# nv-tlabs/DefTet

Measured on AMD Instinct MI355X. Metric: M tet-point tests/s (fwd+bwd) at res=70, 100k queries, higher is better.
Workload: dtype f32

## Files before the change

deftet_amd/csrc/point_in_tet.hip:

```cpp
#pragma clang fp contract(off)

#include <stdlib.h>

#include <algorithm>
#include <type_traits>
#include <vector>

#include "common.hpp"

namespace deftet {
namespace pit {

constexpr float kBig = 1048576.0f;
constexpr float kTau = 1.0f / 128.0f;
constexpr float kMargin = 1.0f / 64.0f;
constexpr float kWMin = 9.3132257e-10f;
constexpr int kMiss = 0x7F7F7F7F;
constexpr int kMaxG = 112;
constexpr int kMaxBins = 15 * 1024;
constexpr int kHitOverflow = -2;

constexpr int kHitPad = 64;
__host__ __device__ inline int hit_pad(int B) { return (B + kHitPad - 1) / kHitPad * kHitPad; }
__host__ __device__ inline size_t hit_cnt_off(int B, int T) { return (size_t)B * T * 2; }
// ... 215 lines not shown
    const float cells = fmaxf(4096.0f, (float)Q * (1.0f / 32.0f)) * layers / fmaxf((float)Q, 1.0f);
    return cells >= 2.0e9f ? 0x7FFFFFFF : (int)cells;
}
__device__ __forceinline__ bool wide_tet(int cx0, int cx1, int cy0, int cy1, int cz0, int cz1, const Grid &g)
{
    return (cx1 - cx0 + 1) * ((cy1 - cy0 + 1) * (cz1 - cz0 + 1)) > g.wide;
}

__device__ __forceinline__ bool query_regular(float x, float y, float z)
{
    return fabsf(x) <= kBig && fabsf(y) <= kBig && fabsf(z) <= kBig;
}

__host__ __device__ inline int table_pitch(int G) { return G + 3; }
__device__ __forceinline__ unsigned table_off(int cz, int cx, int cy, int Gx, int Gp)
{
    return (unsigned)((cz * (Gx + 1) + cx) * Gp + cy);
}

__global__ __launch_bounds__(256) void k_query_bbox(const float *__restrict__ pts, int Q, float *part, int *counters,
                                                    int *result, int nB, long long nQ)
{
    __shared__ float sh[4][6];
    const int b = blockIdx.y;
    {
        const long long nblk = (long long)gridDim.x * gridDim.y, bid = (long long)blockIdx.y * gridDim.x + blockIdx.x;
        const long long i = bid * blockDim.x + threadIdx.x, stride = nblk * blockDim.x;
        if (i < nB * 8) counters[i] = 0;
        for (long long j = i; j < nQ; j += stride) result[j] = kMiss;
    }
    const float *p = pts + (size_t)b * Q * 3;
    float lo[3] = {INFINITY, INFINITY, INFINITY}, hi[3] = {-INFINITY, -INFINITY, -INFINITY};
    constexpr int kBoxKeep = 8;
    const int stride = gridDim.x * blockDim.x;
    for (int q0 = blockIdx.x * blockDim.x + threadIdx.x; q0 < Q; q0 += stride * kBoxKeep) {
        float x[kBoxKeep], y[kBoxKeep], z[kBoxKeep];
#pragma unroll
        for (int k = 0; k < kBoxKeep; ++k) {
            const float *pq = p + (size_t)min(q0 + k * stride, Q - 1) * 3;
            x[k] = pq[0]; y[k] = pq[1]; z[k] = pq[2];
        }
#pragma unroll
        for (int k = 0; k < kBoxKeep; ++k)
            if (query_regular(x[k], y[k], z[k])) {
                lo[0] = fminf(lo[0], x[k]); lo[1] = fminf(lo[1], y[k]); lo[2] = fminf(lo[2], z[k]);
                hi[0] = fmaxf(hi[0], x[k]); hi[1] = fmaxf(hi[1], y[k]); hi[2] = fmaxf(hi[2], z[k]);
            }
    }
#pragma unroll
    for (int off = 32; off > 0; off >>= 1) {
#pragma unroll
        for (int k = 0; k < 3; ++k) {
            lo[k] = fminf(lo[k], __shfl_xor(lo[k], off));
            hi[k] = fmaxf(hi[k], __shfl_xor(hi[k], off));
        }
    }
    const int w = threadIdx.x >> 6;
    if ((threadIdx.x & 63) == 0) {
#pragma unroll
        for (int k = 0; k < 3; ++k) { sh[w][k] = lo[k]; sh[w][3 + k] = hi[k]; }
    }
    __syncthreads();
    if (threadIdx.x < 6) {
        const int k = threadIdx.x;
        float v = sh[0][k];
        for (int i = 1; i < 4; ++i) v = k < 3 ? fminf(v, sh[i][k]) : fmaxf(v, sh[i][k]);
        part[((size_t)b * kBoxBlocks + blockIdx.x) * 6 + k] = v;
    }
}

__device__ __forceinline__ int2 shape_block(int pin)
{
    if (!pin) return make_int2(blockIdx.y, blockIdx.x);
    const int L = blockIdx.y * gridDim.x + blockIdx.x, nB = gridDim.y;
    return make_int2(L % nB, L / nB);
}
static inline int pin_shapes(int Q) { return (size_t)Q * 36 <= ((size_t)4 << 20); }

constexpr int kMaxRowBlocks = 256;
#ifndef PIT_ROWTILE
#define PIT_ROWTILE 2048
#endif
constexpr int kRowTile = PIT_ROWTILE;
constexpr int kLocalKeep = kRowTile / 256;
constexpr int kSub = 8;
constexpr int kParts = 4;
constexpr int kSubPerPart = kSub / kParts;
constexpr int kMaxBin1 = kMaxG * kSub;

template <bool HINT>
__global__ __launch_bounds__(256) void k_slab_local(const float *__restrict__ pts, int Q, const float *__restrict__ bboxPart,
                                                    float *gparam, int G, int Gx, int nblk, int nblkPad, int chunkQ,
                                                    float4 *localQ, int *pre, int *counters, int *irregQ,
                                                    const float *__restrict__ boxIn, float *partOut, int *irrCnt, int *result)
{
    __shared__ int hist[kMaxBin1 + 1];
    __shared__ int wtot[4];
    __shared__ int s_irr, s_out;
    __shared__ float s_box[4][6];
    const int b = blockIdx.y, blk = blockIdx.x, R1 = G * kSub, tid = threadIdx.x;
    const int q0 = blk * chunkQ, q1 = min(Q, q0 + chunkQ);
    const bool keep = chunkQ <= kRowTile;
    float3 kp[kLocalKeep];
    if (keep) {
#pragma unroll
        for (int k = 0; k < kLocalKeep; ++k) {
            const float *p = pts + ((size_t)b * Q + max(min(q0 + tid + k * 256, q1 - 1), 0)) * 3;
            kp[k] = make_float3(p[0], p[1], p[2]);
        }
    }
    if (HINT) {
        for (int q = q0 + tid; q < q1; q += 256) result[(size_t)b * Q + q] = kMiss;
        if (tid == 0) { s_irr = 0; s_out = 0; }
    }
    const Grid g = HINT ? hint_grid(boxIn + (size_t)b * 6, G, Gx) : reduce_grid(bboxPart + (size_t)b * kBoxBlocks * 6, kBoxBlocks, G, Gx);
    float blo[3] = {INFINITY, INFINITY, INFINITY}, bhi[3] = {-INFINITY, -INFINITY, -INFINITY};
    auto box_add = [&](float x, float y, float z) {
        if (HINT && query_regular(x, y, z)) {
            blo[0] = fminf(blo[0], x); blo[1] = fminf(blo[1], y); blo[2] = fminf(blo[2], z);
            bhi[0] = fmaxf(bhi[0], x); bhi[1] = fmaxf(bhi[1], y); bhi[2] = fmaxf(bhi[2], z);
        }
    };
    auto binned = [&](float x, float y, float z) { return HINT ? query_binned(x, y, z, g) : query_regular(x, y, z); };
    auto list_irregular = [&](int q, float x, float y, float z) {
        if (HINT) {
            irregQ[(size_t)b * Q + q0 + atomicAdd(&s_irr, 1)] = q;
            if (query_regular(x, y, z)) atomicAdd(&s_out, 1);
        } else {
            irregQ[(size_t)b * Q + atomicAdd(&counters[b * 4 + 1], 1)] = q;
        }
    };
    if (blk == 0 && tid == 0) {
        float *gp = gparam + b * kGridWords;
#pragma unroll
        for (int k = 0; k < 3; ++k) { gp[k] = g.o[k]; gp[3 + k] = g.inv[k]; gp[6 + k] = g.lo[k]; gp[9 + k] = g.hi[k]; gp[12 + k] = g.pe[k]; gp[15 + k] = g.cs[k]; }
        gp[18] = __int_as_float(wide_cells(g, Q, G, Gx));
        gp[19] = HINT ? 1.0f : 0.f;
    }
    for (int i = tid; i <= R1; i += 256) hist[i] = 0;
    __syncthreads();
    const float rcpG = 1.0f / (float)G;
    int kbin[kLocalKeep], krank[kLocalKeep];
    auto bin_of = [&](float x, float y, float z) {
        const int cy = cell_of(y, g.o[1], g.inv[1], G);
        return cell_of(z, g.o[2], g.inv[2], G) * kSub + (int)(((float)(cy * kSub) + 0.5f) * rcpG);
    };
    if (keep) {
#pragma unroll
        for (int k = 0; k < kLocalKeep; ++k) {
            const int q = q0 + tid + k * 256;
            kbin[k] = -1;
            if (q < q1) {
                box_add(kp[k].x, kp[k].y, kp[k].z);
                if (binned(kp[k].x, kp[k].y, kp[k].z)) {
                    kbin[k] = bin_of(kp[k].x, kp[k].y, kp[k].z);
                    krank[k] = atomicAdd(&hist[kbin[k]], 1);
                } else {
                    list_irregular(q, kp[k].x, kp[k].y, kp[k].z);
                }
            }
        }
    } else {
        for (int q = q0 + tid; q < q1; q += 256) {
            const float *p = pts + ((size_t)b * Q + q) * 3;
            const float x = p[0], y = p[1], z = p[2];
            box_add(x, y, z);
            if (binned(x, y, z)) atomicAdd(&hist[bin_of(x, y, z)], 1);
            else list_irregular(q, x, y, z);
        }
    }
    if (HINT) {
#pragma unroll
        for (int off = 32; off > 0; off >>= 1) {
#pragma unroll
            for (int k = 0; k < 3; ++k) {
                blo[k] = fminf(blo[k], __shfl_xor(blo[k], off));
                bhi[k] = fmaxf(bhi[k], __shfl_xor(bhi[k], off));
            }
        }
        if ((tid & 63) == 0) {
#pragma unroll
            for (int k = 0; k < 3; ++k) { s_box[tid >> 6][k] = blo[k]; s_box[tid >> 6][3 + k] = bhi[k]; }
        }
    }
    __syncthreads();
    if (HINT) {
        if (tid < 6) {
            float v = s_box[0][tid];
            for (int i = 1; i < 4; ++i) v = tid < 3 ? fminf(v, s_box[i][tid]) : fmaxf(v, s_box[i][tid]);
            partOut[((size_t)b * kMaxRowBlocks + blk) * 6 + tid] = v;
        }
        if (tid == 0) {
            irrCnt[b * kMaxRowBlocks + blk] = s_irr;
            irrCnt[(gridDim.y + b) * kMaxRowBlocks + blk] = s_out;
        }
    }
    {
        constexpr int kPer = (kMaxBin1 + 255) / 256;
        const int per = (R1 + 255) / 256, i0 = tid * per;
        int n[kPer], sum = 0;
#pragma unroll
        for (int j = 0; j < kPer; ++j) {
            n[j] = (j < per && i0 + j < R1) ? hist[i0 + j] : 0;
            sum += n[j];
        }
        int incl = sum;
        const int lane = tid & 63, w = tid >> 6;
#pragma unroll
        for (int off = 1; off < 64; off <<= 1) {
            const int t = __shfl_up(incl, off);
            if (lane >= off) incl += t;
        }
        if (lane == 63) wtot[w] = incl;
        __syncthreads();
        int run = incl - sum;
#pragma unroll
        for (int k = 0; k < 4; ++k)
            if (k < w) run += wtot[k];
        int *col = pre + (size_t)b * (R1 + 1) * nblkPad + blk;
#pragma unroll
        for (int j = 0; j < kPer; ++j)
            if (j < per && i0 + j < R1) {
                hist[i0 + j] = run;
                col[(size_t)(i0 + j) * nblkPad] = run;
                run += n[j];
            }
        if (tid == 255) col[(size_t)R1 * nblkPad] = run;
    }
    __syncthreads();
    float4 *dst = localQ + (size_t)b * Q + q0;
    if (keep) {
#pragma unroll
        for (int k = 0; k < kLocalKeep; ++k)
            if (kbin[k] >= 0) dst[hist[kbin[k]] + krank[k]] = make_float4(kp[k].x, kp[k].y, kp[k].z, __int_as_float(q0 + tid + k * 256));
    } else {
        for (int q = q0 + tid; q < q1; q += 256) {
            const float *p = pts + ((size_t)b * Q + q) * 3;
            const float x = p[0], y = p[1], z = p[2];
            if (binned(x, y, z)) dst[atomicAdd(&hist[bin_of(x, y, z)], 1)] = make_float4(x, y, z, __int_as_float(q));
        }
    }
}

#ifndef PIT_SORT_THREADS
#define PIT_SORT_THREADS 256
#endif
constexpr int kSortThreads = PIT_SORT_THREADS;
constexpr int kSortKeep = 1024 / kSortThreads;
constexpr int kRunsPer = kMaxRowBlocks / kSortThreads;
static_assert(kRunsPer * kSortThreads == kMaxRowBlocks && kSortThreads % 64 == 0, "every chunk run has a thread");
__global__ __launch_bounds__(kSortThreads) void k_slab_sort(const float4 *__restrict__ localQ, int Q, const float *__restrict__ gparam,
                                                            int G, int Gx, const int *__restrict__ pre, int nblk, int nblkPad,
                                                            int chunkQ, long long cellStride, int *table, float4 *sortedQ, int pin,
                                                            const float *__restrict__ boxPart, int nPart, int partStride, float *boxOut,
                                                            int hint, const int *__restrict__ irrCnt, int *irregQ, int *counters,
                                                            int *missOut)
{
    if (shape_block(pin).y == 0 && (boxOut || hint)) {
        const int b0 = shape_block(pin).x, nB = gridDim.y;
        if (boxOut && threadIdx.x < 64) {
            float lo[3], hi[3];
            reduce_box(boxPart + (size_t)b0 * partStride * 6, nPart, lo, hi);
            if (threadIdx.x == 0) {
#pragma unroll
                for (int k = 0; k < 3; ++k) { boxOut[b0 * 6 + k] = lo[k]; boxOut[b0 * 6 + 3 + k] = hi[k]; }
            }
        }
        if (hint && threadIdx.x < 64) {
            int n = 0, nOut = 0;
            for (int c = 0; c < nblk; ++c) {
                const int cnt = irrCnt[b0 * kMaxRowBlocks + c];
                nOut += irrCnt[(nB + b0) * kMaxRowBlocks + c];
                const int *src = irregQ + (size_t)b0 * Q + (size_t)c * chunkQ;
                for (int i = (int)threadIdx.x; i < cnt; i += 64) {
                    const int v = src[i];
                    irregQ[(size_t)b0 * Q + n + i] = v;
                }
                n += cnt;
            }
            if (threadIdx.x == 0) {
                counters[b0 * 4 + 0] = 0; counters[b0 * 4 + 1] = n; counters[b0 * 4 + 2] = 0; counters[b0 * 4 + 3] = 0;
#pragma unroll
                for (int k = 0; k < 4; ++k) counters[nB * 4 + b0 * 4 + k] = 0;
                if (missOut) missOut[b0] = nOut;
            }
        }
    }
    extern __shared__ __attribute__((aligned(16))) int cnt[];
    __shared__ int wsum[kSortThreads / 64], wsum2[kSortThreads / 64];
    __shared__ int runStart[kMaxRowBlocks + 1], runSrc[kMaxRowBlocks];
    const int2 sb = shape_block(pin);
    const int b = sb.x, cz = sb.y / kParts, part = sb.y % kParts, tid = threadIdx.x, lane = tid & 63, w = tid >> 6;
    const int GxP = Gx | 1;
    const int cyLo = (part * kSubPerPart * G + kSub - 1) / kSub, cyHi = ((part + 1) * kSubPerPart * G + kSub - 1) / kSub;
    const int nb = (cyHi - cyLo) * GxP, R1 = G * kSub;
    const int binLo = cz * kSub + part * kSubPerPart;
    PHASE_DECL;
    SPAN_MARK(0);
    int a[kRunsPer], len[kRunsPer], asum = 0, lsum = 0;
#pragma unroll
    for (int j = 0; j < kRunsPer; ++j) {
        const int r = tid * kRunsPer + j;
        a[j] = 0; len[j] = 0;
        if (r < nblk) {
            const int *row = pre + (size_t)b * (R1 + 1) * nblkPad;
            a[j] = row[(size_t)binLo * nblkPad + r];
            len[j] = row[(size_t)(binLo + kSubPerPart) * nblkPad + r] - a[j];
        }
        asum += a[j];
        lsum += len[j];
    }
    int s0, n;
    {
        int ia = asum, il = lsum;
#pragma unroll
        for (int off = 1; off < 64; off <<= 1) {
            const int ta = __shfl_up(ia, off), tl = __shfl_up(il, off);
            if (lane >= off) { ia += ta; il += tl; }
        }
        if (lane == 63) { wsum[w] = ia; wsum2[w] = il; }
        __syncthreads();
        int ta = 0, tl = 0, before = 0;
#pragma unroll
        for (int k = 0; k < kSortThreads / 64; ++k) {
            ta += wsum[k];
            tl += wsum2[k];
            if (k < w) before += wsum2[k];
        }
        s0 = ta;
        n = tl;
        int at = before + il - lsum;
#pragma unroll
        for (int j = 0; j < kRunsPer; ++j) {
            const int r = tid * kRunsPer + j;
            if (r < nblk) {
                runStart[r] = at;
                runSrc[r] = r * chunkQ + a[j];
            }
            at += len[j];
        }
        if (tid == 0) runStart[nblk] = n;
    }
    for (int i = tid; i < ((nb + 3) & ~3); i += kSortThreads) cnt[i] = 0;
    __syncthreads();
    const float ox = gparam[b * kGridWords + 0], oy = gparam[b * kGridWords + 1];
    const float ix = gparam[b * kGridWords + 3], iy = gparam[b * kGridWords + 4];
    const int s1 = s0 + n;
    const bool keep = n <= kSortThreads * kSortKeep;
    const float4 *src = localQ + (size_t)b * Q;
    auto source_of = [&](int i) {
        int lo = 0, hi = nblk;
        while (hi - lo > 1) {
            const int mid = (lo + hi) >> 1;
            if (runStart[mid] <= i) lo = mid; else hi = mid;
        }
        return min(runSrc[lo] + (i - runStart[lo]), Q - 1);
    };
    float4 kq[kSortKeep];
    int kbin[kSortKeep], krank[kSortKeep];
    if (keep) {
#pragma unroll
        for (int k = 0; k < kSortKeep; ++k) kq[k] = src[source_of(max(min(tid + k * kSortThreads, n - 1), 0))];
    }
    PHASE_MARK(8);
    if (keep) {
#pragma unroll
        for (int k = 0; k < kSortKeep; ++k) {
            if (tid + k * kSortThreads < n) {
                kbin[k] = (cell_of(kq[k].y, oy, iy, G) - cyLo) * GxP + cell_of(kq[k].x, ox, ix, Gx);
                krank[k] = atomicAdd(&cnt[kbin[k]], 1);
            }
        }
    } else {
        for (int i = tid; i < n; i += kSortThreads) {
            const float4 q = src[source_of(i)];
            atomicAdd(&cnt[(cell_of(q.y, oy, iy, G) - cyLo) * GxP + cell_of(q.x, ox, ix, Gx)], 1);
        }
    }
    __syncthreads();
    PHASE_MARK(9);
    {
        const int nb4 = (nb + 3) >> 2;
        const int per = (nb4 + kSortThreads - 1) / kSortThreads, i0 = min(nb4, tid * per), i1 = min(nb4, i0 + per);
        int4 *c4 = reinterpret_cast<int4 *>(cnt);
        int sum = 0;
        for (int i = i0; i < i1; ++i) {
            const int4 v = c4[i];
            sum += (v.x + v.y) + (v.z + v.w);
        }
        int incl = sum;
#pragma unroll
        for (int off = 1; off < 64; off <<= 1) {
            const int t = __shfl_up(incl, off);
            if (lane >= off) incl += t;
        }
        __syncthreads();
        if (lane == 63) wsum[w] = incl;
        __syncthreads();
        int run = s0 + incl - sum;
#pragma unroll
        for (int k = 0; k < kSortThreads / 64; ++k)
            if (k < w) run += wsum[k];
        for (int i = i0; i < i1; ++i) {
            const int4 v = c4[i];
            int4 o;
            o.x = run; o.y = o.x + v.x; o.z = o.y + v.y; o.w = o.z + v.z;
            run = o.w + v.w;
            c4[i] = o;
        }
    }
    __syncthreads();
    PHASE_MARK(10);
    float4 *dst = sortedQ + (size_t)b * Q;
    if (keep) {
#pragma unroll
        for (int k = 0; k < kSortKeep; ++k)
            if (tid + k * kSortThreads < n) dst[cnt[kbin[k]] + krank[k]] = kq[k];
    }
    PHASE_MARK(11);
    {
        const int Gp = table_pitch(G);
        int *tb = table + (size_t)b * cellStride + (size_t)cz * (Gx + 1) * Gp;
        const int cyEnd = part == kParts - 1 ? Gp : cyHi, ny = cyEnd - cyLo;
        const int total = (Gx + 1) * ny, stepx = kSortThreads / ny, stepy = kSortThreads % ny;
        int cx = tid / ny, ry = tid % ny;
        for (int i = tid; i < total; i += kSortThreads) {
            const int cy = cyLo + ry;
            int v;
            if (cy >= G) v = s1;
            else if (cx < Gx) v = cnt[ry * GxP + cx];
            else v = cy + 1 < cyHi ? cnt[(ry + 1) * GxP] : s1;
            tb[cx * Gp + cy] = v;
            cx += stepx;
            ry += stepy;
            if (ry >= ny) { ry -= ny; ++cx; }
        }
    }
    PHASE_MARK(12);
    SPAN_MARK(1);
    if (keep) return;
    __syncthreads();
    for (int i = tid; i < n; i += kSortThreads) {
        const float4 q = src[source_of(i)];
        dst[atomicAdd(&cnt[(cell_of(q.y, oy, iy, G) - cyLo) * GxP + cell_of(q.x, ox, ix, Gx)], 1)] = q;
    }
// ... 1991 lines not shown
    float c = cond[i];
    if (c < 0) {
        c = 0.f;
        if (clamp_inplace) cond[i] = 0.f;
    }
    out[i] = pred[(size_t)b * T + (long long)c];
}

__global__ __launch_bounds__(256) void k_paste_bwd(const float *__restrict__ cond, const float *__restrict__ gout,
                                                   float *gpred, int T, int Q)
{
    const int b = blockIdx.y;
    const int q = blockIdx.x * blockDim.x + threadIdx.x;
    const bool live = q < Q;
    const size_t i = (size_t)b * Q + (live ? q : 0);
    const float c = live ? cond[i] : 0.f;
    const float g = live ? gout[i] : 0.f;
    const bool miss = live && c < 1.0f;
    float gm = miss ? g : 0.f;
#pragma unroll
    for (int off = 32; off > 0; off >>= 1) gm += __shfl_xor(gm, off);
    __shared__ float wsum[4];
    if ((threadIdx.x & 63) == 0) wsum[threadIdx.x >> 6] = gm;
    __syncthreads();
    if (threadIdx.x == 0) {
        const float tot = (wsum[0] + wsum[1]) + (wsum[2] + wsum[3]);
        if (tot != 0.f) unsafeAtomicAdd(&gpred[(size_t)b * T], tot);
    }
    if (live && !miss) unsafeAtomicAdd(&gpred[(size_t)b * T + (long long)c], g);
}

struct Tunables {
    double gdiv = 6.0;
    double qdiv = 2.0;
    double yzfine = 2.0;
    double xfine = 2.0;
    Tunables()
    {
        auto get = [](const char *name, double lo, double hi, double &dst) {
            if (const char *e = getenv(name)) {
                const double v = atof(e);
                if (v >= lo && v <= hi) dst = v;
            }
        };
        get("DEFTET_PIT_GDIV", 0.25, 4096.0, gdiv);
        get("DEFTET_PIT_QDIV", 0.03, 4096.0, qdiv);
        get("DEFTET_PIT_YZFINE", 0.25, 8.0, yzfine);
        get("DEFTET_PIT_XFINE", 0.25, 16.0, xfine);
    }
};
static const Tunables &tunables()
{
    static const Tunables t;
    return t;
}

static int resolve_auto(int algo, int T, int Q)
{
    if (algo != DEFTET_PIT_AUTO) return algo;
    return (double)Q <= 0.6 * (double)T ? DEFTET_PIT_WAVE : DEFTET_PIT_SLAB;
}

static void pick_grid(int T, int Q, int &G, int &Gx)
{
    const Tunables &tn = tunables();
    const double a = T / tn.gdiv, bq = (Q > 0 ? Q : 1) / tn.qdiv;
    const double m = a < bq ? a : bq;
    long long g = llround(tn.yzfine * cbrt(m < 1 ? 1 : m));
    if (g < 1) g = 1;
    if (g > kMaxG) g = kMaxG;
    long long gx = llround(tn.xfine * (double)g);
    if (gx < 1) gx = 1;
    while (gx > 1 && (g / 4 + 2) * (gx | 1) > kMaxBins) --gx;
    G = (int)g;
    Gx = (int)gx;
}

struct Layout {
    int G, Gx, nRowBlk, chunkQ;
    long long cellStride;
    size_t bytes;
    float *bboxPart, *chunkBox;
    int *irrCnt;
    int nblkPad;
    int *counters, *table, *pre, *result, *irregT, *irregQ;
    float4 *localQ, *sortedQ;
    float *rec, *gparam;
};

static Layout make_layout(int B, int T, int Q, int algo, void *ws, size_t wsBytes)
{
    Layout L{};
    Arena A(ws, wsBytes);
    L.result = A.take<int>((size_t)B * Q);
    if (algo == DEFTET_PIT_BRUTE) {
        L.rec = A.take<float>((size_t)B * T * 32);
    } else {
        pick_grid(T, Q, L.G, L.Gx);
        const long long n = (long long)L.G * (L.Gx + 1) * table_pitch(L.G);
        L.cellStride = (n + 63) / 64 * 64;
        L.nRowBlk = (Q + kRowTile - 1) / kRowTile;
        if (L.nRowBlk > kMaxRowBlocks) L.nRowBlk = kMaxRowBlocks;
        if (L.nRowBlk < 1) L.nRowBlk = 1;
        L.chunkQ = ((Q + L.nRowBlk - 1) / L.nRowBlk + 255) / 256 * 256;
        L.bboxPart = A.take<float>((size_t)B * kBoxBlocks * 6);
        L.chunkBox = A.take<float>((size_t)B * kMaxRowBlocks * 6);
        L.irrCnt = A.take<int>((size_t)B * kMaxRowBlocks * 2);
        L.counters = A.take<int>((size_t)B * (8 + kOvfCap));
        L.gparam = A.take<float>((size_t)B * kGridWords);
        L.table = A.take<int>((size_t)B * L.cellStride);
        L.nblkPad = (L.nRowBlk + 15) / 16 * 16;
        L.pre = A.take<int>((size_t)B * (L.G * kSub + 1) * L.nblkPad);
        L.localQ = A.take<float4>((size_t)B * Q);
        L.sortedQ = A.take<float4>((size_t)B * Q);
        L.irregT = A.take<int>((size_t)B * T);
        L.irregQ = A.take<int>((size_t)B * Q);
    }
    L.bytes = align_up(A.off, 256);
    return L;
}

}
}

using namespace deftet;
using namespace deftet::pit;

extern "C" size_t deftet_point_in_tet_workspace_bytes(int B, int T, int Q, int algo)
{
    if (B <= 0 || T < 0 || Q < 0) return 0;
    return make_layout(B, T, Q, algo, nullptr, 0).bytes;
}

extern "C" size_t deftet_point_in_tet_hits_ints(int B, int T, int Q)
{
    if (B <= 0 || T < 0 || Q < 0) return 0;
    return hit_spill_off(B, T, Q) + (size_t)B * T * 4;
}

extern "C" int deftet_point_in_tet_resolve_algo(int algo, int T, int Q) { return resolve_auto(algo, T, Q); }

extern "C" int deftet_point_in_tet_grid_dims(int T, int Q, int *G_yz, int *G_x)
{
    DEFTET_CHECK_ARG(T >= 0 && Q >= 0 && G_yz && G_x, "bad argument");
    pick_grid(T, Q, *G_yz, *G_x);
    return DEFTET_OK;
}

static int pit_check(const float *tet, const float *pts, const float *cond, const float *bary, const float *pred, const float *occ,
                     const int32_t *hit_buf, int B, int T, int Q, int algo, const void *workspace)
{
    DEFTET_CHECK_ARG(!hit_buf || (((uintptr_t)hit_buf & 15) == 0 && algo != DEFTET_PIT_BRUTE), "hit_buf must be 16-byte aligned and needs a binned algo");
    DEFTET_CHECK_ARG((pred == nullptr) == (occ == nullptr), "pred and occ must be given together");
    DEFTET_CHECK_ARG(!occ || T > 0, "paste_occ needs at least one tet");
    DEFTET_CHECK_ARG(B >= 0 && T >= 0 && Q >= 0, "negative size (B=%d T=%d Q=%d)", B, T, Q);
    DEFTET_CHECK_ARG(algo == DEFTET_PIT_AUTO || algo == DEFTET_PIT_BRUTE || algo == DEFTET_PIT_EXACT || algo == DEFTET_PIT_SLAB || algo == DEFTET_PIT_WAVE || algo == DEFTET_PIT_PAIR, "unknown algo %d", algo);
    if (T >= (1 << 24)) return set_error(DEFTET_ELIMIT, "n_tet=%d does not fit a float-encoded index (2^24)", T);
    DEFTET_CHECK_ARG(B <= 65535, "n_batch=%d exceeds the grid-y limit 65535", B);
    if (Q >= (1 << 27)) return set_error(DEFTET_ELIMIT, "n_query=%d: 16-byte query records are addressed with 32-bit byte offsets (limit 2^27)", Q);
    if (B == 0 || Q == 0) return DEFTET_OK;
    DEFTET_CHECK_ARG(pts && cond, "null pts/cond pointer");
    DEFTET_CHECK_ARG(T == 0 || tet, "null tet pointer");
    DEFTET_CHECK_ARG(((uintptr_t)tet & 15) == 0, "tet must be 16-byte aligned");
    DEFTET_CHECK_ARG(!bary || ((uintptr_t)bary & 15) == 0, "bary must be 16-byte aligned");
    DEFTET_CHECK_ARG(workspace && ((uintptr_t)workspace & 255) == 0, "workspace null or not 256-byte aligned");
    return DEFTET_OK;
}

static int pit_prepare(const Layout &L, const float *pts, int B, int Q, hipStream_t st, const float *boxIn = nullptr, float *boxOut = nullptr,
                       int32_t *missOut = nullptr)
{
    const dim3 blk(256);
    if (boxIn) {
        DEFTET_LAUNCH(k_slab_local<true>, dim3(L.nRowBlk, B), blk, st, pts, Q, L.bboxPart, L.gparam, L.G, L.Gx, L.nRowBlk, L.nblkPad, L.chunkQ,
                      L.localQ, L.pre, L.counters, L.irregQ, boxIn, L.chunkBox, L.irrCnt, L.result);
    } else {
        DEFTET_LAUNCH(k_query_bbox, dim3(kBoxBlocks, B), blk, st, pts, Q, L.bboxPart, L.counters, L.result, B, (long long)B * Q);
        DEFTET_LAUNCH(k_slab_local<false>, dim3(L.nRowBlk, B), blk, st, pts, Q, L.bboxPart, L.gparam, L.G, L.Gx, L.nRowBlk, L.nblkPad, L.chunkQ,
                      L.localQ, L.pre, L.counters, L.irregQ, (const float *)nullptr, (float *)nullptr, (int *)nullptr, (int *)nullptr);
    }
    const size_t shm = align_up((size_t)((L.G + kParts - 1) / kParts + 1) * (L.Gx | 1) * sizeof(int), 16);
    DEFTET_LAUNCH_SHM(k_slab_sort, dim3(L.G * kParts, B), dim3(kSortThreads), shm, st, L.localQ, Q, L.gparam, L.G, L.Gx, L.pre, L.nRowBlk, L.nblkPad,
                      L.chunkQ, L.cellStride, L.table, L.sortedQ, (size_t)Q * 16 <= ((size_t)4 << 20),
                      (const float *)(boxIn ? L.chunkBox : L.bboxPart), boxIn ? L.nRowBlk : kBoxBlocks, boxIn ? kMaxRowBlocks : kBoxBlocks, boxOut,
                      boxIn ? 1 : 0, (const int *)L.irrCnt, L.irregQ, L.counters, (int *)(boxIn ? missOut : nullptr));
    return DEFTET_OK;
}

template <class TS>
static int pit_scan(const Layout &L, typename TS::Arg tet, const float *pts, float *cond, float *bary, const float *pred, float *occ,
                    int32_t *hit_buf, int B, int T, int Q, int algo, hipStream_t st, const int32_t *order = nullptr)
{
    const dim3 blk(256);
    const dim3 gf((Q + 256 * PIT_FIN_QPT - 1) / (256 * PIT_FIN_QPT), B), gt((((T + 255) / 256 + 7) / 8) * 8, B);
    int *ucount = hit_buf ? hit_buf + hit_cnt_off(B, T) : nullptr;
    if (T > 0) {
        if (algo == DEFTET_PIT_EXACT) {
            DEFTET_LAUNCH(k_tet_scan<TS>, gt, blk, st, tet, T, Q, L.gparam, L.G, L.Gx, L.table, L.cellStride, L.sortedQ, L.result,
                          L.counters, L.irregT, (int2 *)hit_buf, pts, L.irregQ, ucount, hit_pad(B), hit_buf ? (int4 *)(hit_buf + hit_spill_off(B, T, Q)) : (int4 *)nullptr);
        } else {
            int4 *spill = hit_buf ? (int4 *)(hit_buf + hit_spill_off(B, T, Q)) : (int4 *)nullptr;
            const int kern = resolve_auto(algo, T, Q);
            const bool slab = kern == DEFTET_PIT_SLAB;
#if PIT_PROBE_SCATTER && PIT_PROBE_PREFILL
            if (spill) DEFTET_HIP(hipMemsetAsync(spill, 0, (size_t)B * Q * 24, st));
#endif
            const dim3 bw(kWvThreads);
            const dim3 gw((((T + kWvThreads - 1) / kWvThreads + 7) / 8) * 8, B);
            const dim3 gp(((((T + 1) / 2 + kWvThreads - 1) / kWvThreads + 7) / 8) * 8, B);
#define PIT_SCAN_ARGS tet, T, Q, L.gparam, L.G, L.Gx, L.table, L.cellStride, L.sortedQ, L.result, L.counters, L.irregT, (int2 *)hit_buf, pts, \
                      L.irregQ, ucount, hit_pad(B), spill, (const int *)order
            typedef TetCfg<TS, true> Ord;
            typedef TetCfg<TS, false> Plain;
            if (slab && order) DEFTET_LAUNCH(k_tet_scan_slab<Ord>, gt, blk, st, PIT_SCAN_ARGS);
            else if (slab) DEFTET_LAUNCH(k_tet_scan_slab<Plain>, gt, blk, st, PIT_SCAN_ARGS);
            else if (kern == DEFTET_PIT_PAIR && order) DEFTET_LAUNCH(k_tet_scan_pair<Ord>, gp, bw, st, PIT_SCAN_ARGS);
            else if (kern == DEFTET_PIT_PAIR) DEFTET_LAUNCH(k_tet_scan_pair<Plain>, gp, bw, st, PIT_SCAN_ARGS);
            else if (order) DEFTET_LAUNCH(k_tet_scan_wave<Ord>, gw, bw, st, PIT_SCAN_ARGS);
            else DEFTET_LAUNCH(k_tet_scan_wave<Plain>, gw, bw, st, PIT_SCAN_ARGS);
#undef PIT_SCAN_ARGS
        }
    } else if (ucount) {
        DEFTET_HIP(hipMemsetAsync(ucount, 0, (size_t)3 * hit_pad(B) * 4, st));
    }
    DEFTET_LAUNCH(k_finalize<TS>, gf, blk, st, tet, pts, T, Q, L.result, cond, bary, pred, occ, (const int2 *)hit_buf, ucount,
                  hit_buf ? hit_buf + hit_list_off(B, T) : nullptr, L.counters, L.irregT, hit_pad(B), pin_shapes(Q), (const float *)L.gparam);
    return DEFTET_OK;
}

template <class TS>
static int pit_forward_checked(typename TS::Arg tet, const float *pts, float *cond, float *bary, const float *pred, float *occ,
                               int32_t *hit_buf, int B, int T, int Q, int algo, void *workspace, size_t workspace_bytes, void *stream_,
                               const int32_t *order, const float *boxIn, float *boxOut, int32_t *missOut)
{
    Layout L = make_layout(B, T, Q, algo, workspace, workspace_bytes);
    DEFTET_CHECK_ARG(L.bytes <= workspace_bytes, "workspace too small: need %zu bytes, got %zu", L.bytes, workspace_bytes);
    hipStream_t st = as_stream(stream_);
    if (algo == DEFTET_PIT_BRUTE) {
        const dim3 blk(256), gq((Q + 255) / 256, B);
        if (T > 0) {
            long long n = (long long)B * T;
            DEFTET_LAUNCH(k_prep_records<TS>, dim3((unsigned)((n + 255) / 256)), blk, st, tet, n, L.rec, T);
        }
        DEFTET_LAUNCH(k_brute, gq, blk, st, L.rec, pts, T, Q, L.result);
        DEFTET_LAUNCH(k_finalize<TS>, dim3((Q + 256 * PIT_FIN_QPT - 1) / (256 * PIT_FIN_QPT), B), blk, st, tet, pts, T, Q, L.result, cond, bary, pred, occ, (const int2 *)nullptr, (int *)nullptr,
                      (int *)nullptr, (const int *)nullptr, L.irregT, 0, pin_shapes(Q), (const float *)nullptr);
        return DEFTET_OK;
    }
    const int rc = pit_prepare(L, pts, B, Q, st, boxIn, boxOut, missOut);
    if (rc != DEFTET_OK) return rc;
    return pit_scan<TS>(L, tet, pts, cond, bary, pred, occ, hit_buf, B, T, Q, algo, st, order);
}
static int pit_forward(const float *tet, const float *pts, float *cond, float *bary, const float *pred, float *occ, int32_t *hit_buf,
                       int B, int T, int Q, int algo, void *workspace, size_t workspace_bytes, void *stream_, const int32_t *order,
                       const float *boxIn = nullptr, float *boxOut = nullptr, int32_t *missOut = nullptr)
{
    int rc = pit_check(tet, pts, cond, bary, pred, occ, hit_buf, B, T, Q, algo, workspace);
    if (rc != DEFTET_OK || B == 0 || Q == 0) return rc;
    return pit_forward_checked<DenseTets>(tet, pts, cond, bary, pred, occ, hit_buf, B, T, Q, algo, workspace, workspace_bytes, stream_, order,
                                          boxIn, boxOut, missOut);
}

extern "C" int deftet_point_in_tet_f32(const float *tet, const float *pts, float *cond, float *bary, const float *pred,
                                       float *occ, int32_t *hit_buf, int B, int T, int Q, int algo, void *workspace,
                                       size_t workspace_bytes, void *stream_)
// ... 2 lines not shown
}

extern "C" int deftet_point_in_tet_ex_f32(const float *tet, const float *pts, float *cond, float *bary, const float *pred,
                                          float *occ, int32_t *hit_buf, int B, int T, int Q, int algo, const int32_t *tet_order,
                                          const float *query_box_in, float *query_box_out, int32_t *query_box_misses,
                                          void *workspace, size_t workspace_bytes, void *stream_)
{
    DEFTET_CHECK_ARG(!query_box_in || query_box_in != query_box_out, "query_box_in and query_box_out must not alias");
    return pit_forward(tet, pts, cond, bary, pred, occ, hit_buf, B, T, Q, algo, workspace, workspace_bytes, stream_, tet_order,
                       query_box_in, query_box_out, query_box_misses);
}

static int pit_prepare_entry(const float *pts, int B, int T, int Q, int algo, void *workspace, size_t workspace_bytes, void *stream_,
                             const float *boxIn, float *boxOut, int32_t *missOut);
extern "C" int deftet_point_in_tet_prepare_f32(const float *pts, int B, int T, int Q, int algo, void *workspace,
                                               size_t workspace_bytes, void *stream_)
{
    return pit_prepare_entry(pts, B, T, Q, algo, workspace, workspace_bytes, stream_, nullptr, nullptr, nullptr);
}
extern "C" int deftet_point_in_tet_prepare_ex_f32(const float *pts, int B, int T, int Q, int algo, const float *query_box_in,
                                                  float *query_box_out, int32_t *query_box_misses, void *workspace,
                                                  size_t workspace_bytes, void *stream_)
{
    DEFTET_CHECK_ARG(!query_box_in || query_box_in != query_box_out, "query_box_in and query_box_out must not alias");
    return pit_prepare_entry(pts, B, T, Q, algo, workspace, workspace_bytes, stream_, query_box_in, query_box_out, query_box_misses);
}
static int pit_prepare_entry(const float *pts, int B, int T, int Q, int algo, void *workspace, size_t workspace_bytes, void *stream_,
                             const float *boxIn, float *boxOut, int32_t *missOut)
{
    DEFTET_CHECK_ARG(B >= 0 && T >= 0 && Q >= 0 && B <= 65535, "bad size (B=%d T=%d Q=%d)", B, T, Q);
    DEFTET_CHECK_ARG(algo == DEFTET_PIT_AUTO || algo == DEFTET_PIT_EXACT || algo == DEFTET_PIT_SLAB || algo == DEFTET_PIT_WAVE || algo == DEFTET_PIT_PAIR, "prepare needs a binned algo (got %d)", algo);
    if (Q >= (1 << 27)) return set_error(DEFTET_ELIMIT, "n_query=%d exceeds 2^27", Q);
    if (B == 0 || Q == 0) return DEFTET_OK;
    DEFTET_CHECK_ARG(pts, "null pts pointer");
    DEFTET_CHECK_ARG(workspace && ((uintptr_t)workspace & 255) == 0, "workspace null or not 256-byte aligned");
    Layout L = make_layout(B, T, Q, algo, workspace, workspace_bytes);
    DEFTET_CHECK_ARG(L.bytes <= workspace_bytes, "workspace too small: need %zu bytes, got %zu", L.bytes, workspace_bytes);
    return pit_prepare(L, pts, B, Q, as_stream(stream_), boxIn, boxOut, missOut);
}

static int pit_scan_entry(const float *tet, const float *pts, float *cond, float *bary, const float *pred, float *occ, int32_t *hit_buf,
                          int B, int T, int Q, int algo, void *workspace, size_t workspace_bytes, void *stream_, const int32_t *order)
{
    DEFTET_CHECK_ARG(algo != DEFTET_PIT_BRUTE, "scan needs a binned algo");
    int rc = pit_check(tet, pts, cond, bary, pred, occ, hit_buf, B, T, Q, algo, workspace);
    if (rc != DEFTET_OK || B == 0 || Q == 0) return rc;
    Layout L = make_layout(B, T, Q, algo, workspace, workspace_bytes);
    DEFTET_CHECK_ARG(L.bytes <= workspace_bytes, "workspace too small: need %zu bytes, got %zu", L.bytes, workspace_bytes);
    return pit_scan<DenseTets>(L, tet, pts, cond, bary, pred, occ, hit_buf, B, T, Q, algo, as_stream(stream_), order);
}

extern "C" int deftet_point_in_tet_scan_f32(const float *tet, const float *pts, float *cond, float *bary, const float *pred,
                                            float *occ, int32_t *hit_buf, int B, int T, int Q, int algo, void *workspace,
                                            size_t workspace_bytes, void *stream_)
{
    return pit_scan_entry(tet, pts, cond, bary, pred, occ, hit_buf, B, T, Q, algo, workspace, workspace_bytes, stream_, nullptr);
}

extern "C" int deftet_point_in_tet_scan_ex_f32(const float *tet, const float *pts, float *cond, float *bary, const float *pred,
                                                    float *occ, int32_t *hit_buf, int B, int T, int Q, int algo,
                                                    const int32_t *tet_order, void *workspace, size_t workspace_bytes, void *stream_)
{
    return pit_scan_entry(tet, pts, cond, bary, pred, occ, hit_buf, B, T, Q, algo, workspace, workspace_bytes, stream_, tet_order);
}

extern "C" int deftet_point_in_tet_read_stats(const void *workspace, size_t workspace_bytes, int B, int T, int Q, int algo,
                                              int32_t *out_host, void *stream_)
{
    DEFTET_CHECK_ARG(workspace && out_host && B > 0 && algo != DEFTET_PIT_BRUTE, "bad argument");
    Layout L = make_layout(B, T, Q, algo, const_cast<void *>(workspace), workspace_bytes);
    DEFTET_CHECK_ARG(L.bytes <= workspace_bytes, "workspace too small");
    hipStream_t st = as_stream(stream_);
    std::vector<int32_t> tmp((size_t)B * 8);
    DEFTET_HIP(hipMemcpyAsync(tmp.data(), L.counters, (size_t)B * 32, hipMemcpyDeviceToHost, st));
    DEFTET_HIP(hipStreamSynchronize(st));
    for (int b = 0; b < B; ++b)
        for (int k = 0; k < 4; ++k) {
            out_host[b * 8 + k] = tmp[(size_t)b * 4 + k];
            out_host[b * 8 + 4 + k] = tmp[(size_t)B * 4 + (size_t)b * 4 + k];
        }
    return DEFTET_OK;
}

#ifdef PIT_PHASE_TIMING
extern "C" int deftet_debug_occupancy(int *out8)
{
    int n = 0;
    DEFTET_HIP(hipOccupancyMaxActiveBlocksPerMultiprocessor(&n, (const void *)deftet::pit::k_tet_scan_wave<deftet::pit::TetCfg<deftet::pit::DenseTets, false>>, 256, 0)); out8[0] = n;
    DEFTET_HIP(hipOccupancyMaxActiveBlocksPerMultiprocessor(&n, (const void *)deftet::pit::k_tet_scan_pair<deftet::pit::TetCfg<deftet::pit::DenseTets, false>>, 256, 0)); out8[1] = n;
    DEFTET_HIP(hipOccupancyMaxActiveBlocksPerMultiprocessor(&n, (const void *)deftet::pit::k_tet_scan_slab<deftet::pit::TetCfg<deftet::pit::DenseTets, false>>, 256, 0)); out8[2] = n;
    hipFuncAttributes a;
    DEFTET_HIP(hipFuncGetAttributes(&a, (const void *)deftet::pit::k_tet_scan_wave<deftet::pit::TetCfg<deftet::pit::DenseTets, false>>));
    out8[3] = (int)a.sharedSizeBytes; out8[4] = a.numRegs; out8[5] = (int)a.maxDynamicSharedSizeBytes;
    hipDeviceProp_t pr;
    DEFTET_HIP(hipGetDeviceProperties(&pr, 0));
    out8[6] = (int)pr.sharedMemPerMultiprocessor; out8[7] = (int)pr.sharedMemPerBlock;
    return DEFTET_OK;
}
extern "C" int deftet_debug_span_read(unsigned long long *out, int n_waves)
{
    DEFTET_CHECK_ARG(out && n_waves > 0 && n_waves <= deftet::pit::kPhaseWaves, "bad argument");
    DEFTET_HIP(hipMemcpyFromSymbol(out, HIP_SYMBOL(deftet::pit::g_span), (size_t)n_waves * 16));
    return DEFTET_OK;
}
extern "C" int deftet_debug_reason_read(unsigned long long *out8, int reset)
{
    DEFTET_HIP(hipMemcpyFromSymbol(out8, HIP_SYMBOL(deftet::pit::g_reason), 64));
    if (reset) {
        unsigned long long z[8] = {0};
        DEFTET_HIP(hipMemcpyToSymbol(HIP_SYMBOL(deftet::pit::g_reason), z, 64));
    }
    return DEFTET_OK;
}
extern "C" int deftet_debug_phase_read(unsigned long long *out16, int reset)
{
    std::vector<unsigned long long> h((size_t)kPhaseWaves * 16);
    DEFTET_HIP(hipMemcpyFromSymbol(h.data(), HIP_SYMBOL(deftet::pit::g_phase), h.size() * sizeof(unsigned long long)));
    for (int i = 0; i < 16; ++i) out16[i] = 0;
    for (size_t w = 0; w < (size_t)kPhaseWaves; ++w)
        for (int i = 0; i < 16; ++i) out16[i] += h[w * 16 + i];
    if (reset) {
        std::fill(h.begin(), h.end(), 0ull);
        DEFTET_HIP(hipMemcpyToSymbol(HIP_SYMBOL(deftet::pit::g_phase), h.data(), h.size() * sizeof(unsigned long long)));
    }
    return DEFTET_OK;
}
#endif

constexpr long long kDenseQueriesPerTet = 2;
extern "C" size_t deftet_point_in_tet_bwd_workspace_bytes(int B, int T, int Q)
{
    if (B <= 0 || T < 0 || Q < 0) return 0;
    const size_t lists = align_up((size_t)B * T * 4, 256) + align_up((size_t)B * Q * 4, 256) + align_up((size_t)B * 4, 256);
    const size_t miss = align_up((size_t)B * kMissStride * 4, 256);
    return lists > miss ? lists : miss;
}

static bool tets_null(const float *tet) { return tet == nullptr; }
static bool tets_null(const IndexedTets &s) { return s.pos == nullptr || s.idx == nullptr; }
static bool tets_misaligned(const float *tet) { return ((uintptr_t)tet & 15) != 0; }
static bool tets_misaligned(const IndexedTets &s) { return ((uintptr_t)s.idx & 15) != 0 || ((uintptr_t)s.pos & 3) != 0; }

template <class TS>
static int pit_bwd(typename TS::Arg tet, const float *pts, const float *cond, const float *grad_w, float *grad_tet, float *grad_pts,
                   const float *grad_occ, float *grad_pred, const int32_t *hit_buf, int B, int T, int Q, int accumulate, void *workspace,
                   size_t workspace_bytes, void *stream_)
{
    DEFTET_CHECK_ARG(B >= 0 && T >= 0 && Q >= 0, "negative size");
    DEFTET_CHECK_ARG(B <= 65535, "n_batch=%d exceeds 65535", B);
    DEFTET_CHECK_ARG((grad_occ == nullptr) == (grad_pred == nullptr), "grad_occ and grad_pred must be given together");
    hipStream_t st = as_stream(stream_);
    if (B == 0) return DEFTET_OK;
    if (grad_pts && Q > 0) DEFTET_HIP(hipMemsetAsync(grad_pts, 0, (size_t)B * Q * 12, st));
    if (T == 0) return DEFTET_OK;
    DEFTET_CHECK_ARG(grad_tet && ((uintptr_t)grad_tet & 15) == 0, "grad_tet null or not 16-byte aligned");
    if (Q == 0) {
        if (!accumulate) {
            DEFTET_HIP(hipMemsetAsync(grad_tet, 0, (size_t)B * T * 48, st));
            if (grad_pred) DEFTET_HIP(hipMemsetAsync(grad_pred, 0, (size_t)B * T * 4, st));
        }
        return DEFTET_OK;
    }
    DEFTET_CHECK_ARG(!tets_null(tet) && pts && cond && grad_w, "null pointer");
    DEFTET_CHECK_ARG(!tets_misaligned(tet) && ((uintptr_t)grad_w & 15) == 0, "tet/grad_w must be 16-byte aligned");
    const bool dense = (long long)Q > kDenseQueriesPerTet * (long long)T && workspace && ((uintptr_t)workspace & 255) == 0 &&
                       workspace_bytes >= deftet_point_in_tet_bwd_workspace_bytes(B, T, Q);
// ... 218 lines not shown
```

Baseline: 1.059 billion.

## Widen slab-local blocks, halve sub-bins, make prefix table row-major, split box block

The slab-local binning kernel now runs 512 threads per block, and the number of y sub-bins per z slab drops from 8 to 4. The per-chunk prefix table moves from a column-major, padded-block layout to a row-per-chunk layout with a 32-aligned pitch, so each chunk writes contiguous rows while the sort kernel does strided gathers. The bounding-box and irregular-count reduction moves to a dedicated extra block row in the sort grid, which returns early, and redundant keep-loads are skipped. These changes aim to cut sort-stage contention and improve write coalescing. The cost is coarser bins, which may leave more work per sort bin, and one extra block per batch.

```diff
diff --git a/deftet_amd/csrc/point_in_tet.hip b/deftet_amd/csrc/point_in_tet.hip
--- a/deftet_amd/csrc/point_in_tet.hip
+++ b/deftet_amd/csrc/point_in_tet.hip
@@ -321,22 +321,28 @@
 #define PIT_ROWTILE 2048
 #endif
 constexpr int kRowTile = PIT_ROWTILE;
-constexpr int kLocalKeep = kRowTile / 256;
-constexpr int kSub = 8;
+#ifndef PIT_LOCAL_THREADS
+#define PIT_LOCAL_THREADS 512
+#endif
+constexpr int kLocalThreads = PIT_LOCAL_THREADS;
+constexpr int kLocalWaves = kLocalThreads / 64;
+constexpr int kLocalKeep = kRowTile / kLocalThreads;
+static_assert(kLocalThreads % 64 == 0 && kLocalKeep * kLocalThreads == kRowTile, "whole waves, whole trips over a chunk");
+constexpr int kSub = 4;
 constexpr int kParts = 4;
 constexpr int kSubPerPart = kSub / kParts;
 constexpr int kMaxBin1 = kMaxG * kSub;
 
 template <bool HINT>
-__global__ __launch_bounds__(256) void k_slab_local(const float *__restrict__ pts, int Q, const float *__restrict__ bboxPart,
-                                                    float *gparam, int G, int Gx, int nblk, int nblkPad, int chunkQ,
+__global__ __launch_bounds__(kLocalThreads) void k_slab_local(const float *__restrict__ pts, int Q, const float *__restrict__ bboxPart,
+                                                    float *gparam, int G, int Gx, int nblk, int prePitch, int chunkQ,
                                                     float4 *localQ, int *pre, int *counters, int *irregQ,
                                                     const float *__restrict__ boxIn, float *partOut, int *irrCnt, int *result)
 {
     __shared__ int hist[kMaxBin1 + 1];
-    __shared__ int wtot[4];
+    __shared__ int wtot[kLocalWaves];
     __shared__ int s_irr, s_out;
-    __shared__ float s_box[4][6];
+    __shared__ float s_box[kLocalWaves][6];
     const int b = blockIdx.y, blk = blockIdx.x, R1 = G * kSub, tid = threadIdx.x;
     const int q0 = blk * chunkQ, q1 = min(Q, q0 + chunkQ);
     const bool keep = chunkQ <= kRowTile;
@@ -344,12 +350,12 @@
     if (keep) {
 #pragma unroll
         for (int k = 0; k < kLocalKeep; ++k) {
-            const float *p = pts + ((size_t)b * Q + max(min(q0 + tid + k * 256, q1 - 1), 0)) * 3;
+            const float *p = pts + ((size_t)b * Q + max(min(q0 + tid + k * kLocalThreads, q1 - 1), 0)) * 3;
             kp[k] = make_float3(p[0], p[1], p[2]);
         }
     }
     if (HINT) {
-        for (int q = q0 + tid; q < q1; q += 256) result[(size_t)b * Q + q] = kMiss;
+        for (int q = q0 + tid; q < q1; q += kLocalThreads) result[(size_t)b * Q + q] = kMiss;
         if (tid == 0) { s_irr = 0; s_out = 0; }
     }
     const Grid g = HINT ? hint_grid(boxIn + (size_t)b * 6, G, Gx) : reduce_grid(bboxPart + (size_t)b * kBoxBlocks * 6, kBoxBlocks, G, Gx);
@@ -376,7 +382,7 @@
         gp[18] = __int_as_float(wide_cells(g, Q, G, Gx));
         gp[19] = HINT ? 1.0f : 0.f;
     }
-    for (int i = tid; i <= R1; i += 256) hist[i] = 0;
+    for (int i = tid; i <= R1; i += kLocalThreads) hist[i] = 0;
     __syncthreads();
     const float rcpG = 1.0f / (float)G;
     int kbin[kLocalKeep], krank[kLocalKeep];
@@ -387,7 +393,7 @@
     if (keep) {
 #pragma unroll
         for (int k = 0; k < kLocalKeep; ++k) {
-            const int q = q0 + tid + k * 256;
+            const int q = q0 + tid + k * kLocalThreads;
             kbin[k] = -1;
             if (q < q1) {
                 box_add(kp[k].x, kp[k].y, kp[k].z);
@@ -400,7 +406,7 @@
             }
         }
     } else {
-        for (int q = q0 + tid; q < q1; q += 256) {
+        for (int q = q0 + tid; q < q1; q += kLocalThreads) {
             const float *p = pts + ((size_t)b * Q + q) * 3;
             const float x = p[0], y = p[1], z = p[2];
             box_add(x, y, z);
@@ -426,7 +432,7 @@
     if (HINT) {
         if (tid < 6) {
             float v = s_box[0][tid];
-            for (int i = 1; i < 4; ++i) v = tid < 3 ? fminf(v, s_box[i][tid]) : fmaxf(v, s_box[i][tid]);
+            for (int i = 1; i < kLocalWaves; ++i) v = tid < 3 ? fminf(v, s_box[i][tid]) : fmaxf(v, s_box[i][tid]);
             partOut[((size_t)b * kMaxRowBlocks + blk) * 6 + tid] = v;
         }
         if (tid == 0) {
@@ -435,8 +441,8 @@
         }
     }
     {
-        constexpr int kPer = (kMaxBin1 + 255) / 256;
-        const int per = (R1 + 255) / 256, i0 = tid * per;
+        constexpr int kPer = (kMaxBin1 + kLocalThreads - 1) / kLocalThreads;
+        const int per = (R1 + kLocalThreads - 1) / kLocalThreads, i0 = tid * per;
         int n[kPer], sum = 0;
 #pragma unroll
         for (int j = 0; j < kPer; ++j) {
@@ -454,26 +460,26 @@
         __syncthreads();
         int run = incl - sum;
 #pragma unroll
-        for (int k = 0; k < 4; ++k)
+        for (int k = 0; k < kLocalWaves; ++k)
             if (k < w) run += wtot[k];
-        int *col = pre + (size_t)b * (R1 + 1) * nblkPad + blk;
+        int *row = pre + ((size_t)b * nblk + blk) * prePitch;
 #pragma unroll
         for (int j = 0; j < kPer; ++j)
             if (j < per && i0 + j < R1) {
                 hist[i0 + j] = run;
-                col[(size_t)(i0 + j) * nblkPad] = run;
+                row[i0 + j] = run;
                 run += n[j];
             }
-        if (tid == 255) col[(size_t)R1 * nblkPad] = run;
+        if (tid == kLocalThreads - 1) row[R1] = run;
     }
     __syncthreads();
     float4 *dst = localQ + (size_t)b * Q + q0;
     if (keep) {
 #pragma unroll
         for (int k = 0; k < kLocalKeep; ++k)
-            if (kbin[k] >= 0) dst[hist[kbin[k]] + krank[k]] = make_float4(kp[k].x, kp[k].y, kp[k].z, __int_as_float(q0 + tid + k * 256));
+            if (kbin[k] >= 0) dst[hist[kbin[k]] + krank[k]] = make_float4(kp[k].x, kp[k].y, kp[k].z, __int_as_float(q0 + tid + k * kLocalThreads));
     } else {
-        for (int q = q0 + tid; q < q1; q += 256) {
+        for (int q = q0 + tid; q < q1; q += kLocalThreads) {
             const float *p = pts + ((size_t)b * Q + q) * 3;
             const float x = p[0], y = p[1], z = p[2];
             if (binned(x, y, z)) dst[atomicAdd(&hist[bin_of(x, y, z)], 1)] = make_float4(x, y, z, __int_as_float(q));
@@ -489,13 +495,13 @@
 constexpr int kRunsPer = kMaxRowBlocks / kSortThreads;
 static_assert(kRunsPer * kSortThreads == kMaxRowBlocks && kSortThreads % 64 == 0, "every chunk run has a thread");
 __global__ __launch_bounds__(kSortThreads) void k_slab_sort(const float4 *__restrict__ localQ, int Q, const float *__restrict__ gparam,
-                                                            int G, int Gx, const int *__restrict__ pre, int nblk, int nblkPad,
+                                                            int G, int Gx, const int *__restrict__ pre, int nblk, int prePitch,
                                                             int chunkQ, long long cellStride, int *table, float4 *sortedQ, int pin,
                                                             const float *__restrict__ boxPart, int nPart, int partStride, float *boxOut,
                                                             int hint, const int *__restrict__ irrCnt, int *irregQ, int *counters,
                                                             int *missOut)
 {
-    if (shape_block(pin).y == 0 && (boxOut || hint)) {
+    if (shape_block(pin).y == 0) {
         const int b0 = shape_block(pin).x, nB = gridDim.y;
         if (boxOut && threadIdx.x < 64) {
             float lo[3], hi[3];
@@ -524,15 +530,17 @@
                 if (missOut) missOut[b0] = nOut;
             }
         }
+        return;
     }
     extern __shared__ __attribute__((aligned(16))) int cnt[];
     __shared__ int wsum[kSortThreads / 64], wsum2[kSortThreads / 64];
     __shared__ int runStart[kMaxRowBlocks + 1], runSrc[kMaxRowBlocks];
-    const int2 sb = shape_block(pin);
+    const int2 sb0 = shape_block(pin);
+    const int2 sb = make_int2(sb0.x, sb0.y - 1);
     const int b = sb.x, cz = sb.y / kParts, part = sb.y % kParts, tid = threadIdx.x, lane = tid & 63, w = tid >> 6;
     const int GxP = Gx | 1;
     const int cyLo = (part * kSubPerPart * G + kSub - 1) / kSub, cyHi = ((part + 1) * kSubPerPart * G + kSub - 1) / kSub;
-    const int nb = (cyHi - cyLo) * GxP, R1 = G * kSub;
+    const int nb = (cyHi - cyLo) * GxP;
     const int binLo = cz * kSub + part * kSubPerPart;
     PHASE_DECL;
     SPAN_MARK(0);
@@ -542,9 +550,9 @@
         const int r = tid * kRunsPer + j;
         a[j] = 0; len[j] = 0;
         if (r < nblk) {
-            const int *row = pre + (size_t)b * (R1 + 1) * nblkPad;
-            a[j] = row[(size_t)binLo * nblkPad + r];
-            len[j] = row[(size_t)(binLo + kSubPerPart) * nblkPad + r] - a[j];
+            const int *row = pre + ((size_t)b * nblk + r) * prePitch + binLo;
+            a[j] = row[0];
+            len[j] = row[kSubPerPart] - a[j];
         }
         asum += a[j];
         lsum += len[j];
@@ -599,7 +607,9 @@
     int kbin[kSortKeep], krank[kSortKeep];
     if (keep) {
 #pragma unroll
-        for (int k = 0; k < kSortKeep; ++k) kq[k] = src[source_of(max(min(tid + k * kSortThreads, n - 1), 0))];
+        for (int k = 0; k < kSortKeep; ++k)
+            if (k == 0 || k * kSortThreads < n)
+                kq[k] = src[source_of(max(min(tid + k * kSortThreads, n - 1), 0))];
     }
     PHASE_MARK(8);
     if (keep) {
@@ -2757,7 +2767,7 @@
     size_t bytes;
     float *bboxPart, *chunkBox;
     int *irrCnt;
-    int nblkPad;
+    int prePitch;
     int *counters, *table, *pre, *result, *irregT, *irregQ;
     float4 *localQ, *sortedQ;
     float *rec, *gparam;
@@ -2784,8 +2794,8 @@
         L.counters = A.take<int>((size_t)B * (8 + kOvfCap));
         L.gparam = A.take<float>((size_t)B * kGridWords);
         L.table = A.take<int>((size_t)B * L.cellStride);
-        L.nblkPad = (L.nRowBlk + 15) / 16 * 16;
-        L.pre = A.take<int>((size_t)B * (L.G * kSub + 1) * L.nblkPad);
+        L.prePitch = (L.G * kSub + 1 + 31) / 32 * 32;
+        L.pre = A.take<int>((size_t)B * L.nRowBlk * L.prePitch);
         L.localQ = A.take<float4>((size_t)B * Q);
         L.sortedQ = A.take<float4>((size_t)B * Q);
         L.irregT = A.take<int>((size_t)B * T);
@@ -2845,17 +2855,17 @@
 static int pit_prepare(const Layout &L, const float *pts, int B, int Q, hipStream_t st, const float *boxIn = nullptr, float *boxOut = nullptr,
                        int32_t *missOut = nullptr)
 {
-    const dim3 blk(256);
+    const dim3 blk(256), lblk(kLocalThreads);
     if (boxIn) {
-        DEFTET_LAUNCH(k_slab_local<true>, dim3(L.nRowBlk, B), blk, st, pts, Q, L.bboxPart, L.gparam, L.G, L.Gx, L.nRowBlk, L.nblkPad, L.chunkQ,
+        DEFTET_LAUNCH(k_slab_local<true>, dim3(L.nRowBlk, B), lblk, st, pts, Q, L.bboxPart, L.gparam, L.G, L.Gx, L.nRowBlk, L.prePitch, L.chunkQ,
                       L.localQ, L.pre, L.counters, L.irregQ, boxIn, L.chunkBox, L.irrCnt, L.result);
     } else {
         DEFTET_LAUNCH(k_query_bbox, dim3(kBoxBlocks, B), blk, st, pts, Q, L.bboxPart, L.counters, L.result, B, (long long)B * Q);
-        DEFTET_LAUNCH(k_slab_local<false>, dim3(L.nRowBlk, B), blk, st, pts, Q, L.bboxPart, L.gparam, L.G, L.Gx, L.nRowBlk, L.nblkPad, L.chunkQ,
+        DEFTET_LAUNCH(k_slab_local<false>, dim3(L.nRowBlk, B), lblk, st, pts, Q, L.bboxPart, L.gparam, L.G, L.Gx, L.nRowBlk, L.prePitch, L.chunkQ,
                       L.localQ, L.pre, L.counters, L.irregQ, (const float *)nullptr, (float *)nullptr, (int *)nullptr, (int *)nullptr);
     }
     const size_t shm = align_up((size_t)((L.G + kParts - 1) / kParts + 1) * (L.Gx | 1) * sizeof(int), 16);
-    DEFTET_LAUNCH_SHM(k_slab_sort, dim3(L.G * kParts, B), dim3(kSortThreads), shm, st, L.localQ, Q, L.gparam, L.G, L.Gx, L.pre, L.nRowBlk, L.nblkPad,
+    DEFTET_LAUNCH_SHM(k_slab_sort, dim3(L.G * kParts + 1, B), dim3(kSortThreads), shm, st, L.localQ, Q, L.gparam, L.G, L.Gx, L.pre, L.nRowBlk, L.prePitch,
                       L.chunkQ, L.cellStride, L.table, L.sortedQ, (size_t)Q * 16 <= ((size_t)4 << 20),
                       (const float *)(boxIn ? L.chunkBox : L.bboxPart), boxIn ? L.nRowBlk : kBoxBlocks, boxIn ? kMaxRowBlocks : kBoxBlocks, boxOut,
                       boxIn ? 1 : 0, (const int *)L.irrCnt, L.irregQ, L.counters, (int *)(boxIn ? missOut : nullptr));
@@ -3024,6 +3034,16 @@
     return DEFTET_OK;
 }
 
+extern "C" int deftet_debug_point_in_tet_layout(int B, int T, int Q, int algo, long long *out8)
+{
+    DEFTET_CHECK_ARG(out8 && B > 0 && T >= 0 && Q >= 0 && algo != DEFTET_PIT_BRUTE, "bad argument");
+    const Layout L = make_layout(B, T, Q, algo, nullptr, 0);
+    auto off = [](const void *p) { return (long long)reinterpret_cast<uintptr_t>(p); };
+    out8[0] = L.G; out8[1] = L.Gx; out8[2] = L.cellStride;
+    out8[3] = off(L.gparam); out8[4] = off(L.table); out8[5] = off(L.sortedQ); out8[6] = off(L.counters); out8[7] = off(L.irregQ);
+    return DEFTET_OK;
+}
+
 #ifdef PIT_PHASE_TIMING
 extern "C" int deftet_debug_occupancy(int *out8)
 {
```

Result: faster. 1.072 billion, median of 6 (+1.2%).
